# worldlife123/cbench_BaSIC

Hardware: AMD Instinct MI355X
Metric: encode+decode Mpix/s (higher is better)
Workload: dtype f32; 1 GPU; hyperprior codec N=128 M=192 (lossy_graph_scalable_exp_hp), synthetic 3x256x256 images (image i = manual_seed(i), rand), 256 images per GPU per step resident in HBM, compress+decompress incl. bitstream D2H/H2D, 6 concurrent stream workers per GPU (step k on worker k mod W: whole batches, W in flight); images_per_gpu=256, workers=6, rans_waves_per_workgroup=8, batches_in_flight=6, parallelism=image-sharded x1, RCCL all-reduce of metric sums

## Files before the change

### cbench_basic_amd/csrc/conv.hip

```cpp
#include "common.h"

#include <cstdlib>
#include <cstring>
#include <new>
#include <vector>

using namespace basic;

namespace {
thread_local bool g_dynamic_tiles = false;
}
namespace basic {
bool set_dynamic_tiles(bool on)
{
    const bool prev = g_dynamic_tiles;
    g_dynamic_tiles = on;
    return prev;
}
}

namespace {

typedef float f32x16 __attribute__((ext_vector_type(16)));
typedef float f32x4 __attribute__((ext_vector_type(4)));
// ... 1 lines not shown
constexpr int kFewTaps = 9;
constexpr int kVeryFewTaps = 6;
constexpr int stage_channels(int ntaps, int waves)
{
    return (ntaps > kFewTaps ? 2 : (ntaps > kVeryFewTaps ? 4 : 8)) * (waves == 8 ? 2 : 1);
}
constexpr int plan_waves(int mt, int ntaps) { return (mt == 4 && ntaps > kFewTaps) ? 8 : 4; }
constexpr int kMaxTaps = 25;
constexpr int kTilePos = 128;
constexpr int kPSlots = 12;
constexpr int kPSlotsNarrow = 24;
constexpr int patch_slots(int mt) { return mt <= 2 ? kPSlotsNarrow : kPSlots; }
constexpr int kPSlotsFused = 6;
constexpr int kFusedCK = 4;
constexpr int kMaxCoutPerLaunch = 192;
constexpr int kSplitBelowBlocks = 384;
constexpr int kPackTail = 32 * 32 * 8 + 2048;

struct TapLaunch {
    const float *in;
    float *out;
    const float *wpack;
    const float *wrow;
    const float *bias;
    int64_t split_wstride;
    const float *gammaT;
    const float *beta;
    int batch, cin, cin_pad, cout, coutp;
    int out_ctotal, co_base;
    int in_h, in_w, out_h, out_w;
// ... 325 lines not shown
            }
    }
}

typedef __bf16 bf16x8 __attribute__((ext_vector_type(8)));
typedef unsigned u32x4 __attribute__((ext_vector_type(4)));

constexpr int kSplitWaves = 8;
constexpr int kSplitThreads = 64 * kSplitWaves;
constexpr int kSplitCK = 16;
constexpr int kSplitStageTaps = 5;
constexpr int kSplitBlockU4 = 4 * 3 * 64;
constexpr int kSplitStageU4 = kSplitStageTaps * kSplitBlockU4;
constexpr int kSplitWSlots = (kSplitStageU4 + kSplitThreads - 1) / kSplitThreads;
static_assert(kSplitWSlots % 2 == 0, "weight stage in two halves");
constexpr size_t kSplitLdsBytes = 2 * kSplitStageU4 * 16 + 2 * 128 * sizeof(float);

__device__ __forceinline__ void split_bf16x3(const float (&x)[8], u32x4 &p0, u32x4 &p1, u32x4 &p2)
{
#pragma unroll
    for (int i = 0; i < 4; ++i) {
        const unsigned a = __float_as_uint(x[2 * i]), b = __float_as_uint(x[2 * i + 1]);
        const unsigned a0 = a & 0xFFFF0000u, b0 = b & 0xFFFF0000u;
        p0[i] = (a >> 16) | b0;
        const unsigned ra = __float_as_uint(x[2 * i] - __uint_as_float(a0)), rb = __float_as_uint(x[2 * i + 1] - __uint_as_float(b0));
        const unsigned a1 = ra & 0xFFFF0000u, b1 = rb & 0xFFFF0000u;
        p1[i] = (ra >> 16) | b1;
        const unsigned sa = __float_as_uint(__uint_as_float(ra) - __uint_as_float(a1)), sb = __float_as_uint(__uint_as_float(rb) - __uint_as_float(b1));
        p2[i] = (sa >> 16) | (sb & 0xFFFF0000u);
    }
}

__device__ __forceinline__ f32x16 mfma_bf16(const u32x4 &a, const u32x4 &b, const f32x16 &c)
{
    return __builtin_amdgcn_mfma_f32_32x32x16_bf16(__builtin_bit_cast(bf16x8, a), __builtin_bit_cast(bf16x8, b), c, 0, 0, 0);
}

constexpr int kSplitPatchPos = 416;
constexpr int kSplitPieceBytes = kSplitPatchPos * 32;
constexpr size_t kSplitLdsPatchBytes = kSplitLdsBytes + 3 * kSplitPieceBytes;
static_assert(kSplitLdsPatchBytes <= 160 * 1024, "patch beside the weight stages");
static_assert(kSplitLdsBytes % 16 == 0, "16-byte aligned patch");
constexpr int kSplitPatchRounds = (2 * kSplitPatchPos + kSplitThreads - 1) / kSplitThreads;

template <int KH, int KW, int KWB, bool PATCH>
__global__ __launch_bounds__(kSplitThreads, 1) void conv_split_bf16_kernel(const TapLaunch g, const u32x4 *wsplit)
{
    constexpr int MT = 4;
    constexpr int kTapsA = KH * KW, kTapsAll = KH * (KW + KWB);
    constexpr int kGroups = kTapsAll / kSplitStageTaps;
    static_assert(kTapsAll % kSplitStageTaps == 0, "taps per channel block must be whole stages");
    static_assert(KWB > 0 && KWB <= KW, "fused phases: second grid inside the first");
    extern __shared__ u32x4 lds_u4[];
    float *chan_const = reinterpret_cast<float *>(lds_u4 + 2 * kSplitStageU4);

    const int tid = threadIdx.x;
    const int lane = tid & 63;
    const int khalf = lane >> 5;
    const int wave = __builtin_amdgcn_readfirstlane(tid >> 6);

    int bid = xcd_tile(blockIdx.x, gridDim.x);
    const int tx_i = bid % g.tiles_x; bid /= g.tiles_x;
    const int ty_i = bid % g.tiles_y; bid /= g.tiles_y;
    const int TB = 1 << g.tb_log, TH = 1 << g.th_log, TW = 1 << g.tw_log;
    const int b0 = bid * TB, my0 = ty_i * TH, mx0 = tx_i * TW;
    struct Pos { int tb, my, mx; };
    auto pos_of = [&](int t) {
        const int qq = (t >> 6) * 32 + (t & 31);
        return Pos{qq >> (g.tw_log + g.th_log), my0 + ((qq >> g.tw_log) & (TH - 1)), mx0 + (qq & (TW - 1))};
    };
    const Pos lp = pos_of(tid);
    const int tb = lp.tb, b = b0 + lp.tb;

    if (tid < 128) {
        chan_const[tid] = g.bias ? g.bias[tid] : 0.f;
        chan_const[128 + tid] = g.beta ? g.beta[tid] : 1.f;
    }

    const int64_t plane = static_cast<int64_t>(g.in_h) * g.in_w;
    const int nimg = (g.batch - b0 < TB) ? g.batch - b0 : TB;
    const __amdgpu_buffer_rsrc_t rsrc = __builtin_amdgcn_make_buffer_rsrc(
        const_cast<float *>(g.in + static_cast<int64_t>(b0) * g.cin * plane), 0, static_cast<int>(nimg * g.cin * plane * 4), 0x00020000);
    const int gy_l = lp.my * g.s_in + g.dymin, gx_l = lp.mx * g.s_in + g.dxmin;
    const int lane_off = static_cast<int>((((static_cast<int64_t>(tb) * g.cin + 8 * khalf) * g.in_h + gy_l) * g.in_w + gx_l) * 4);
    constexpr int kSpanX = KW;
    static_assert(KH * kSpanX <= 32, "one validity bit per tap offset");
    unsigned vmask = 0;
    if (b < g.batch) {
#pragma unroll
        for (int dy = 0; dy < KH; ++dy)
#pragma unroll
            for (int dx = 0; dx < kSpanX; ++dx) {
                const int yy = gy_l + dy, xx = gx_l + dx;
                if (yy >= 0 && yy < g.in_h && xx >= 0 && xx < g.in_w) vmask |= 1u << (dy * kSpanX + dx);
            }
    }
    const int plane_bytes = static_cast<int>(plane * 4);
    auto tap_row = [](int t) { return t < kTapsA ? t / KW : (t - kTapsA) / KWB; };
    auto tap_col = [](int t) { return t < kTapsA ? t % KW : (t - kTapsA) % KWB + (KW - KWB); };
    auto load_b = [&](int cb, int T, float (&d)[8]) __attribute__((always_inline)) {
        const int dy = tap_row(T), dx = tap_col(T);
        const int voff = ((vmask >> (dy * kSpanX + dx)) & 1u) ? lane_off + (dy * g.in_w + dx) * 4 : 0x7FFFFFF0;
        const int soff = cb * kSplitCK * plane_bytes;
#pragma unroll
        for (int j = 0; j < 8; ++j)
            d[j] = __builtin_bit_cast(float, __builtin_amdgcn_raw_buffer_load_b32(rsrc, voff, soff + j * plane_bytes, 0));
    };

    const int ncb = g.cin / kSplitCK;
    constexpr int kHalf = kSplitWSlots / 2;
    u32x4 wst[kHalf];
    auto fetch_w = [&](int s, int h) __attribute__((always_inline)) {
        const u32x4 *src = wsplit + static_cast<int64_t>(s) * kSplitStageU4 + tid;
#pragma unroll
        for (int sl = h * kHalf; sl < (h + 1) * kHalf; ++sl)
            if (sl * kSplitThreads + tid < kSplitStageU4) wst[sl - h * kHalf] = src[sl * kSplitThreads];
    };
    auto store_w = [&](int buf, int h) __attribute__((always_inline)) {
        u32x4 *dst = lds_u4 + buf * kSplitStageU4 + tid;
#pragma unroll
        for (int sl = h * kHalf; sl < (h + 1) * kHalf; ++sl)
            if (sl * kSplitThreads + tid < kSplitStageU4) dst[sl * kSplitThreads] = wst[sl - h * kHalf];
    };

    char *const patch = reinterpret_cast<char *>(lds_u4) + kSplitLdsBytes;
    const int PW = TW + KW - 1, PH = TH + KH - 1, npos = TB * PH * PW;
    int pvoff[kSplitPatchRounds], brow[KH];
    if constexpr (PATCH) {
#pragma unroll
        for (int r = 0; r < kSplitPatchRounds; ++r) {
            const int i = r * kSplitThreads + tid, p = i >> 1, h = i & 1;
            const int prow = p / PW, x = p - prow * PW, img = prow / PH, row = prow - img * PH;
            const int gy = my0 + g.dymin + row, gx = mx0 + g.dxmin + x;
            const bool inside = i < 2 * npos && img < nimg && gy >= 0 && gy < g.in_h && gx >= 0 && gx < g.in_w;
            pvoff[r] = inside ? static_cast<int>((((static_cast<int64_t>(img) * g.cin + 8 * h) * g.in_h + gy) * g.in_w + gx) * 4)
                              : 0x7FFFFFF0;
        }
#pragma unroll
        for (int dy = 0; dy < KH; ++dy) brow[dy] = ((tb * PH + (lp.my - my0) + dy) * PW + (lp.mx - mx0)) * 32 + 16 * khalf;
    }
    float pf[kSplitPatchRounds][8];
    auto fetch_patch = [&](int cb) __attribute__((always_inline)) {
        const int soff = cb * kSplitCK * plane_bytes;
#pragma unroll
        for (int r = 0; r < kSplitPatchRounds; ++r)
#pragma unroll
            for (int j = 0; j < 8; ++j)
                pf[r][j] = __builtin_bit_cast(float, __builtin_amdgcn_raw_buffer_load_b32(rsrc, pvoff[r], soff + j * plane_bytes, 0));
    };
    auto store_patch = [&]() __attribute__((always_inline)) {
#pragma unroll
        for (int r = 0; r < kSplitPatchRounds; ++r)
            if (r * kSplitThreads + tid < 2 * npos) {
                u32x4 q[3];
                split_bf16x3(pf[r], q[0], q[1], q[2]);
#pragma unroll
                for (int pc = 0; pc < 3; ++pc)
                    *reinterpret_cast<u32x4 *>(patch + (r * kSplitThreads + tid) * 16 + pc * kSplitPieceBytes) = q[pc];
            }
    };
    auto read_b = [&](int T, u32x4 (&d)[3]) __attribute__((always_inline)) {
        const char *src = patch + brow[tap_row(T)] + 32 * tap_col(T);
#pragma unroll
        for (int pc = 0; pc < 3; ++pc) d[pc] = *reinterpret_cast<const u32x4 *>(src + pc * kSplitPieceBytes);
    };

    f32x16 acc[MT], acc2[MT];
#pragma unroll
    for (int m = 0; m < MT; ++m)
#pragma unroll
        for (int r = 0; r < 16; ++r) {
            acc[m][r] = 0.f;
            acc2[m][r] = 0.f;
        }

    float xb[8];
    u32x4 bq[2][3];
    if constexpr (PATCH) fetch_patch(0);
    else load_b(0, 0, xb);
    fetch_w(0, 0);
    store_w(0, 0);
    fetch_w(0, 1);
    store_w(0, 1);
    if constexpr (PATCH) store_patch();
    for (int cb = 0; cb < ncb; ++cb) {
#pragma unroll
        for (int gi = 0; gi < kGroups; ++gi) {
            const int s = cb * kGroups + gi;
            __syncthreads();
            const bool more = s + 1 < ncb * kGroups;
            if (more) fetch_w(s + 1, 0);
            __builtin_amdgcn_sched_barrier(0);
            const u32x4 *wl = lds_u4 + (s & 1) * kSplitStageU4 + lane;
#pragma unroll
            for (int tl = 0; tl < kSplitStageTaps; ++tl) {
                const int T = gi * kSplitStageTaps + tl;
                float xn[8];
                u32x4 bd[3];
                if constexpr (PATCH) {
                    if (T == 0) read_b(0, bq[0]);
                } else {
                    if (T + 1 < kTapsAll) load_b(cb, T + 1, xn);
                    else load_b(cb + 1 < ncb ? cb + 1 : cb, 0, xn);
                    __builtin_amdgcn_sched_barrier(0);
                    split_bf16x3(xb, bd[0], bd[1], bd[2]);
                }
                const u32x4 (&bp)[3] = PATCH ? bq[T & 1] : bd;
                f32x16 (&dst)[MT] = T < kTapsA ? acc : acc2;
                u32x4 ap[2][3];
#pragma unroll
                for (int pc = 0; pc < 3; ++pc) ap[0][pc] = wl[(tl * MT * 3 + pc) * 64];
#pragma unroll
                for (int m = 0; m < MT; ++m) {
                    const int cur = m & 1;
                    if (m + 1 < MT) {
#pragma unroll
                        for (int pc = 0; pc < 3; ++pc) ap[cur ^ 1][pc] = wl[((tl * MT + m + 1) * 3 + pc) * 64];
                    } else if constexpr (PATCH) {
                        if (T + 1 < kTapsAll) read_b(T + 1, bq[(T + 1) & 1]);
                    }
                    __builtin_amdgcn_sched_barrier(0);
                    dst[m] = mfma_bf16(ap[cur][2], bp[0], dst[m]);
                    dst[m] = mfma_bf16(ap[cur][1], bp[1], dst[m]);
                    dst[m] = mfma_bf16(ap[cur][0], bp[2], dst[m]);
                    dst[m] = mfma_bf16(ap[cur][1], bp[0], dst[m]);
                    dst[m] = mfma_bf16(ap[cur][0], bp[1], dst[m]);
                    dst[m] = mfma_bf16(ap[cur][0], bp[0], dst[m]);
                    __builtin_amdgcn_sched_barrier(0);
                }
                if constexpr (!PATCH) {
#pragma unroll
                    for (int j = 0; j < 8; ++j) xb[j] = xn[j];
                }
                if (tl == 1 && more) {
                    store_w((s + 1) & 1, 0);
                    fetch_w(s + 1, 1);
                    __builtin_amdgcn_sched_barrier(0);
                }
                if constexpr (PATCH) {
                    if (gi == 0 && tl == 1) {
                        fetch_patch(cb + 1 < ncb ? cb + 1 : cb);
                        __builtin_amdgcn_sched_barrier(0);
                    }
                }
                if (tl == 3 && more) store_w((s + 1) & 1, 1);
            }
        }
        if constexpr (PATCH) {
            if (cb + 1 < ncb) {
                __syncthreads();
                store_patch();
            }
        }
    }

    const int tid_e = wave * 64 + static_cast<int>(__lane_id());
    const int khalf_e = (tid_e >> 5) & 1, col_e = tid_e & 31;
    float *gl = reinterpret_cast<float *>(lds_u4);
    const bool gdn = g.act == BASIC_ACT_GDN || g.act == BASIC_ACT_IGDN;
    auto finish = [&](f32x16 (&acc)[MT]) __attribute__((always_inline)) {
        if (g.bias) {
#pragma unroll
            for (int m = 0; m < MT; ++m)
#pragma unroll
                for (int rq = 0; rq < 4; ++rq) {
                    const f32x4 b4 = *reinterpret_cast<const f32x4 *>(chan_const + 32 * m + 8 * rq + 4 * khalf_e);
#pragma unroll
                    for (int e = 0; e < 4; ++e) acc[m][4 * rq + e] += b4[e];
                }
        }
        if (gdn) {
            f32x16 nrm[MT];
#pragma unroll
            for (int m = 0; m < MT; ++m)
#pragma unroll
                for (int r = 0; r < 16; ++r) nrm[m][r] = 0.f;
#pragma unroll
            for (int st = 0; st < 64; ++st) {
                const int kk = 32 * (st >> 4) + 8 * ((st & 15) >> 2) + (st & 3);
                float gk[4];
                load_a<4>(gl + ((kk + 4 * khalf_e) * 32 + col_e) * 4, gk);
                const float x = acc[st >> 4][st & 15];
                const float bfrag = x * x;
#pragma unroll
                for (int m = 0; m < MT; ++m)
                    nrm[m] = __builtin_amdgcn_mfma_f32_32x32x2f32(gk[m], bfrag, nrm[m], 0, 0, 0);
            }
#pragma unroll
            for (int m = 0; m < MT; ++m)
#pragma unroll
                for (int rq = 0; rq < 4; ++rq) {
                    const f32x4 b4 = *reinterpret_cast<const f32x4 *>(chan_const + 128 + 32 * m + 8 * rq + 4 * khalf_e);
#pragma unroll
                    for (int e = 0; e < 4; ++e) {
                        const int r = 4 * rq + e;
                        const float nv = nrm[m][r] + b4[e];
                        acc[m][r] *= (g.act == BASIC_ACT_GDN) ? __builtin_amdgcn_rsqf(nv) : __builtin_amdgcn_sqrtf(nv);
                    }
                }
        }
    };
    if (gdn) {
        __syncthreads();
        const f32x4 *src = reinterpret_cast<const f32x4 *>(g.gammaT);
        f32x4 *dst = reinterpret_cast<f32x4 *>(gl);
#pragma unroll
        for (int sl = 0; sl < 128 * 32 * 4 / 4 / kSplitThreads; ++sl) dst[sl * kSplitThreads + tid_e] = src[sl * kSplitThreads + tid_e];
        __syncthreads();
    }
    finish(acc);
    finish(acc2);

    const Pos ep = pos_of(tid_e);
    const int my = ep.my, mx = ep.mx, be = b0 + ep.tb;
    if (my < g.mh && mx < g.mw && be < g.batch) {
        const int oy = my * g.s_out + g.oy0, ox = mx * g.s_out + g.ox0;
        const int64_t oplane = static_cast<int64_t>(g.out_h) * g.out_w;
        float *o = g.out + (static_cast<int64_t>(be) * g.out_ctotal + g.co_base) * oplane + static_cast<int64_t>(oy) * g.out_w + ox;
#pragma unroll
        for (int m = 0; m < MT; ++m)
#pragma unroll
            for (int r = 0; r < 16; ++r) {
                const int co = 32 * m + 8 * (r >> 2) + 4 * khalf_e + (r & 3);
                if (co < g.cout) {
                    f32x2 v2;
                    v2[0] = apply_act(acc[m][r], g.act);
                    v2[1] = apply_act(acc2[m][r], g.act);
                    *reinterpret_cast<f32x2 *>(o + co * oplane) = v2;
                }
            }
    }
}

template <int KH, bool PATCH>
hipError_t launch_split(const TapLaunch &g, const u32x4 *ws, int blocks, hipStream_t st)
{
    const hipError_t e = ensure_max_lds(reinterpret_cast<const void *>(conv_split_bf16_kernel<KH, 3, 2, PATCH>));
    if (e != hipSuccess) return e;
    hipLaunchKernelGGL((conv_split_bf16_kernel<KH, 3, 2, PATCH>), dim3(blocks), dim3(kSplitThreads),
                       PATCH ? kSplitLdsPatchBytes : kSplitLdsBytes, st, g, ws);
    return hipGetLastError();
}

constexpr int kFirstSlots = 10;

template <bool ROWS>
__global__ __launch_bounds__(512, 1) void conv5x5_cin4_gdn_persistent_kernel(const TapLaunch g, int ntiles, int *sched)
{
    extern __shared__ float lds[];
    constexpr int MT = 4, kCK = ROWS ? 3 : 4, KW = 5, kSteps = ROWS ? 5 * 8 : 25 * 2;
    constexpr int kWFloats = ROWS ? 80 * 32 * 4 : 25 * 4 * 32 * 4;
    constexpr int kGFloats = 128 * 32 * 4;
    float *wl = lds;
    float *gl = lds + kWFloats;
    const int tid = threadIdx.x;
// ... 940 lines not shown
        if (kh == 3 && kw == 3) return launch_one<MT, kFew, 3, 3, WF>(g, blocks, nsplit, lds_bytes, st);
        return launch_one<MT, kFew, 0, 0, WF>(g, blocks, nsplit, lds_bytes, st);
    }
    if (kh == 3 && kw == 2) return launch_one<MT, kVeryFew, 3, 2, WV>(g, blocks, nsplit, lds_bytes, st);
    if (kh == 2 && kw == 3) return launch_one<MT, kVeryFew, 2, 3, WV>(g, blocks, nsplit, lds_bytes, st);
    if (kh == 2 && kw == 2) return launch_one<MT, kVeryFew, 2, 2, WV>(g, blocks, nsplit, lds_bytes, st);
    return launch_one<MT, kVeryFew, 0, 0, WV>(g, blocks, nsplit, lds_bytes, st);
}

int ilog2(int v) { int l = 0; while ((1 << (l + 1)) <= v) ++l; return l; }
int pow2_ceil(int v) { int p = 1; while (p < v) p <<= 1; return p; }

}

namespace {
struct LaunchChoice { bool use_split, fuse_ok, bf16x3, split_patch; };
LaunchChoice choose_launches(const basic_conv_plan *p, int batch, int oh, int ow, const void *d_out)
{
    const int64_t pos_blocks = (static_cast<int64_t>(batch) * ((oh + p->s_out - 1) / p->s_out) * ((ow + p->s_out - 1) / p->s_out) + kTilePos - 1) / kTilePos;
    const char *dbg_env = getenv("BASIC_CONV_DEBUG");
    const int dbg = dbg_env ? atoi(dbg_env) : 0;
    LaunchChoice c;
    c.use_split = !p->split.empty() && !(dbg & 8) && (pos_blocks < kSplitBelowBlocks || (dbg & 4));
    c.fuse_ok = ow % 2 == 0 && (reinterpret_cast<uintptr_t>(d_out) & 7) == 0 && !(dbg & 512);
    const char *f32_env = getenv("BASIC_CONV_F32");
    c.bf16x3 = !(f32_env && atoi(f32_env) != 0);
    c.split_patch = !(dbg & 1024);
    return c;
}
}

extern "C" int basic_conv_plan_launches(const basic_conv_plan *p, int batch, int in_h, int in_w)
{
    int oh = 0, ow = 0;
    if (!p || batch < 1 || basic_conv_plan_out_hw(p, in_h, in_w, &oh, &ow)) return -1;
    if (p->d_wsm) return 1;
    const LaunchChoice c = choose_launches(p, batch, oh, ow, nullptr);
    int n = 0;
    for (const Chunk &ch : (c.use_split ? p->split : p->chunks))
        for (const Phase &ph : ((c.fuse_ok && !ch.fused.empty()) ? ch.fused : ch.phases)) {
            const int mh = (oh - ph.oy0 + p->s_out - 1) / p->s_out, mw = (ow - ph.ox0 + p->s_out - 1) / p->s_out;
            if (mh > 0 && mw > 0) ++n;
// ... 16 lines not shown
        g.tiles_x = (in_w + kSmTileW - 1) / kSmTileW;
        const int blocks = batch * g.tiles_y * g.tiles_x;
        const bool dma_ok = in_w % 4 == 0 && (reinterpret_cast<uintptr_t>(d_in) & 15) == 0;
        if (dma_ok && in_h >= 64) {
            g.tiles_y = (in_h + kSm2TileH - 1) / kSm2TileH;
            hipLaunchKernelGGL(deconv5s2_cout3_dma2_kernel, dim3(batch * g.tiles_y * g.tiles_x), dim3(256), 0, as_stream(hip_stream), g);
        } else if (dma_ok)
            hipLaunchKernelGGL(deconv5s2_cout3_dma_kernel, dim3(blocks), dim3(256), 0, as_stream(hip_stream), g);
        else
            hipLaunchKernelGGL(deconv5s2_cout3_kernel, dim3(blocks), dim3(256), 0, as_stream(hip_stream), g);
        BASIC_HIP_TRY(hipGetLastError());
        return BASIC_OK;
    }
    const LaunchChoice choice = choose_launches(p, batch, oh, ow, d_out);
    const bool use_split = choice.use_split, fuse_ok = choice.fuse_ok;
    for (const Chunk &ch : (use_split ? p->split : p->chunks))
    for (const Phase &ph : ((fuse_ok && !ch.fused.empty()) ? ch.fused : ch.phases)) {
        TapLaunch g{};
        g.in = d_in; g.out = d_out; g.wpack = ph.d_wpack; g.wrow = ph.d_wrow; g.split_wstride = ph.split_wstride; g.bias = ch.d_bias; g.gammaT = p->d_gammaT; g.beta = p->d_beta;
        g.batch = batch; g.cin = p->cin; g.cin_pad = ph.ntaps ? ph.cin_pad : 0; g.cout = ch.cout; g.coutp = ch.coutp; g.out_ctotal = p->cout; g.co_base = ch.co0;
        g.in_h = in_h; g.in_w = in_w; g.out_h = oh; g.out_w = ow;
        g.s_in = p->s_in; g.s_out = p->s_out; g.oy0 = ph.oy0; g.ox0 = ph.ox0;
        g.mh = (oh - ph.oy0 + p->s_out - 1) / p->s_out;
        g.mw = (ow - ph.ox0 + p->s_out - 1) / p->s_out;
        if (g.mh <= 0 || g.mw <= 0) continue;
        g.ntaps = ph.ntaps; g.dymin = ph.dymin; g.dxmin = ph.dxmin;
        std::memcpy(g.dy, ph.dy, sizeof(g.dy));
        std::memcpy(g.dx, ph.dx, sizeof(g.dx));
        g.act = p->act;
        const int kCK = ph.ck;
        if (choice.bf16x3 && ph.d_wsplit) {
            int tw = pow2_ceil(g.mw); if (tw > 16) tw = 16;
            int th = pow2_ceil(g.mh); if (th > kSplitWaves * 32 / tw) th = kSplitWaves * 32 / tw;
            const int tb = kSplitWaves * 32 / (tw * th);
            if (static_cast<int64_t>(tb) * p->cin * in_h * in_w * 4 < (1ll << 31)) {
                g.tw_log = ilog2(tw); g.th_log = ilog2(th); g.tb_log = ilog2(tb);
                g.tiles_y = (g.mh + th - 1) / th;
                g.tiles_x = (g.mw + tw - 1) / tw;
                const int blocks = ((batch + tb - 1) / tb) * g.tiles_y * g.tiles_x;
                hipStream_t st = as_stream(hip_stream);
                const u32x4 *ws = static_cast<const u32x4 *>(ph.d_wsplit);
                BASIC_REQUIRE(ph.kw == 3 && ph.kwb == 2 && (ph.kh == 3 || ph.kh == 2), "conv_forward: split-bf16 plan / kernel instantiation mismatch");
                const bool patch = choice.split_patch && g.s_in == 1 && tb * (th + ph.kh - 1) * (tw + ph.kw - 1) <= kSplitPatchPos;
                const hipError_t e = ph.kh == 3 ? (patch ? launch_split<3, true>(g, ws, blocks, st) : launch_split<3, false>(g, ws, blocks, st))
                                                : (patch ? launch_split<2, true>(g, ws, blocks, st) : launch_split<2, false>(g, ws, blocks, st));
                BASIC_HIP_TRY(e);
                continue;
            }
        }
        int tw = pow2_ceil(g.mw); if (tw > 16) tw = 16;
        const int threads = 64 * ph.waves, tile_pos = 32 * ph.waves;
        int th = pow2_ceil(g.mh); if (th > tile_pos / tw) th = tile_pos / tw;
        int tb = tile_pos / (tw * th);
        const bool first_layer_path = ch.mt == 4 && ch.nsplit == 1 && ph.waves == 8 && ph.kh == 5 && ph.kw == 5 &&
                                      ph.cin_pad == kCK && kCK == 4 && ch.cout == 128 && p->d_gammaT;
        g.ph = (th - 1) * g.s_in + ph.span_y;
        g.pw = (tw - 1) * g.s_in + ph.span_x;
        g.patch4 = (ph.waves == 8 && !first_layer_path && in_w % 4 == 0 && (reinterpret_cast<uintptr_t>(d_in) & 15) == 0) ? 1 : 0;
        g.pwp = g.patch4 ? (g.pw + 3 + 3) / 4 * 4 : (g.pw | 1);
        const int punit = g.patch4 ? 4 : 1;
// ... 18 lines not shown
        hipStream_t st = as_stream(hip_stream);
        if (first_layer_path) {
            const bool rows = ph.d_wrow != nullptr;
            const int patch_pad1 = (tb * (rows ? 3 : kCK) * g.ph * g.pwp + 511) / 512 * 512;
            const size_t lds1 = sizeof(float) * ((rows ? 10240 : 12800) + 16384 + 2 * static_cast<size_t>(patch_pad1) + 256 + 4);
            if (lds1 <= 160 * 1024 && patch_pad1 <= kFirstSlots * 512) {
                BASIC_HIP_TRY(ensure_max_lds(reinterpret_cast<const void *>(conv5x5_cin4_gdn_persistent_kernel<false>)));
                BASIC_HIP_TRY(ensure_max_lds(reinterpret_cast<const void *>(conv5x5_cin4_gdn_persistent_kernel<true>)));
                int dev = 0, cus = 256;
                (void)hipGetDevice(&dev);
                (void)hipDeviceGetAttribute(&cus, hipDeviceAttributeMultiprocessorCount, dev);
                const int grid = blocks < cus ? blocks : cus;
                int *sched = nullptr;
                if (g_dynamic_tiles) {
                    auto *pm = const_cast<basic_conv_plan *>(p);
                    if (!pm->d_sched) BASIC_HIP_TRY(hipMalloc(&pm->d_sched, sizeof(int)));
                    BASIC_HIP_TRY(hipMemsetAsync(pm->d_sched, 0, sizeof(int), st));
                    sched = pm->d_sched;
                }
                if (rows) hipLaunchKernelGGL(conv5x5_cin4_gdn_persistent_kernel<true>, dim3(grid), dim3(512), lds1, st, g, blocks, sched);
                else hipLaunchKernelGGL(conv5x5_cin4_gdn_persistent_kernel<false>, dim3(grid), dim3(512), lds1, st, g, blocks, sched);
                BASIC_HIP_TRY(hipGetLastError());
                continue;
            }
        }
        if (ph.kwb) {
            switch (ch.mt) {
                case 1: rc = launch_fused<1>(g, ph.kh, ph.kw, ph.kwb, ph.ck, ph.waves, blocks, ch.nsplit, lds_bytes, st); break;
                case 2: rc = launch_fused<2>(g, ph.kh, ph.kw, ph.kwb, ph.ck, ph.waves, blocks, ch.nsplit, lds_bytes, st); break;
                case 3: rc = launch_fused<3>(g, ph.kh, ph.kw, ph.kwb, ph.ck, ph.waves, blocks, ch.nsplit, lds_bytes, st); break;
                case 4: rc = launch_fused<4>(g, ph.kh, ph.kw, ph.kwb, ph.ck, ph.waves, blocks, ch.nsplit, lds_bytes, st); break;
// ... 19 lines not shown
```

Before: 827.6 Mpix/s.

## Make split-bf16 conv kernel persistent with atomic dynamic tile scheduling

Turns the split-bf16x3 conv kernel into a persistent kernel launched with at most one block per CU. Each block pulls further tiles through an atomic counter and prefetches the next tile's weights and patch across tile boundaries, so per-block launch and prologue costs are paid once per block rather than once per tile. Weight fetches move to buffer loads, and the LDS layout is reworked to hold a next-tile slot. The price is a memset and atomic counters per plan, shared mutable scheduler state that could race between concurrent streams using the same plan, and a more intricate pipeline.

```diff
diff --git a/cbench_basic_amd/csrc/conv.hip b/cbench_basic_amd/csrc/conv.hip
--- a/cbench_basic_amd/csrc/conv.hip
+++ b/cbench_basic_amd/csrc/conv.hip
@@ -39,6 +39,7 @@
 constexpr int kPSlotsFused = 6;
 constexpr int kFusedCK = 4;
 constexpr int kMaxCoutPerLaunch = 192;
+constexpr int kSchedCounters = 16;
 constexpr int kSplitBelowBlocks = 384;
 constexpr int kPackTail = 32 * 32 * 8 + 2048;
 
@@ -394,7 +395,13 @@
 constexpr int kSplitStageU4 = kSplitStageTaps * kSplitBlockU4;
 constexpr int kSplitWSlots = (kSplitStageU4 + kSplitThreads - 1) / kSplitThreads;
 static_assert(kSplitWSlots % 2 == 0, "weight stage in two halves");
-constexpr size_t kSplitLdsBytes = 2 * kSplitStageU4 * 16 + 2 * 128 * sizeof(float);
+constexpr int kSplitStageBytes = kSplitStageU4 * 16;
+constexpr int kSplitGammaOff = kSplitStageBytes;
+constexpr int kSplitGammaBytes = 128 * 32 * 4 * static_cast<int>(sizeof(float));
+constexpr int kSplitConstBytes = 2 * 128 * static_cast<int>(sizeof(float));
+constexpr int kSplitConstOffDirect = kSplitGammaOff + kSplitGammaBytes;
+constexpr int kSplitSlotOffDirect = kSplitConstOffDirect + kSplitConstBytes;
+constexpr size_t kSplitLdsBytes = kSplitSlotOffDirect + 16;
 
 __device__ __forceinline__ void split_bf16x3(const float (&x)[8], u32x4 &p0, u32x4 &p1, u32x4 &p2)
 {
@@ -418,13 +425,19 @@
 
 constexpr int kSplitPatchPos = 416;
 constexpr int kSplitPieceBytes = kSplitPatchPos * 32;
-constexpr size_t kSplitLdsPatchBytes = kSplitLdsBytes + 3 * kSplitPieceBytes;
+constexpr int kSplitPatchOff = 2 * kSplitStageBytes;
+constexpr int kSplitConstOffPatch = kSplitPatchOff + 3 * kSplitPieceBytes;
+constexpr int kSplitSlotOffPatch = kSplitConstOffPatch - 4;
+constexpr size_t kSplitLdsPatchBytes = kSplitConstOffPatch + kSplitConstBytes;
 static_assert(kSplitLdsPatchBytes <= 160 * 1024, "patch beside the weight stages");
-static_assert(kSplitLdsBytes % 16 == 0, "16-byte aligned patch");
+static_assert(kSplitPatchOff % 16 == 0, "16-byte aligned patch");
+static_assert(kSplitGammaOff + kSplitGammaBytes <= kSplitConstOffPatch, "gamma^T below bias and beta");
 constexpr int kSplitPatchRounds = (2 * kSplitPatchPos + kSplitThreads - 1) / kSplitThreads;
 
+typedef const __attribute__((address_space(4))) TapLaunch *SplitArgs;
+
 template <int KH, int KW, int KWB, bool PATCH>
-__global__ __launch_bounds__(kSplitThreads, 1) void conv_split_bf16_kernel(const TapLaunch g, const u32x4 *wsplit)
+__global__ __launch_bounds__(kSplitThreads, 1) void conv_split_bf16_kernel(const TapLaunch g, const u32x4 *wsplit, int ntiles, int *sched)
 {
     constexpr int MT = 4;
     constexpr int kTapsA = KH * KW, kTapsAll = KH * (KW + KWB);
@@ -432,55 +445,88 @@
     static_assert(kTapsAll % kSplitStageTaps == 0, "taps per channel block must be whole stages");
     static_assert(KWB > 0 && KWB <= KW, "fused phases: second grid inside the first");
     extern __shared__ u32x4 lds_u4[];
-    float *chan_const = reinterpret_cast<float *>(lds_u4 + 2 * kSplitStageU4);
+    char *const lds = reinterpret_cast<char *>(lds_u4);
+    float *chan_const = reinterpret_cast<float *>(lds + (PATCH ? kSplitConstOffPatch : kSplitConstOffDirect));
+    int *const next_slot = reinterpret_cast<int *>(lds + (PATCH ? kSplitSlotOffPatch : kSplitSlotOffDirect));
 
     const int tid = threadIdx.x;
-    const int lane = tid & 63;
-    const int khalf = lane >> 5;
     const int wave = __builtin_amdgcn_readfirstlane(tid >> 6);
-
-    int bid = xcd_tile(blockIdx.x, gridDim.x);
-    const int tx_i = bid % g.tiles_x; bid /= g.tiles_x;
-    const int ty_i = bid % g.tiles_y; bid /= g.tiles_y;
     const int TB = 1 << g.tb_log, TH = 1 << g.th_log, TW = 1 << g.tw_log;
-    const int b0 = bid * TB, my0 = ty_i * TH, mx0 = tx_i * TW;
-    struct Pos { int tb, my, mx; };
-    auto pos_of = [&](int t) {
-        const int qq = (t >> 6) * 32 + (t & 31);
-        return Pos{qq >> (g.tw_log + g.th_log), my0 + ((qq >> g.tw_log) & (TH - 1)), mx0 + (qq & (TW - 1))};
-    };
-    const Pos lp = pos_of(tid);
-    const int tb = lp.tb, b = b0 + lp.tb;
 
     if (tid < 128) {
         chan_const[tid] = g.bias ? g.bias[tid] : 0.f;
         chan_const[128 + tid] = g.beta ? g.beta[tid] : 1.f;
     }
-
+    if (tid == 0) *next_slot = static_cast<int>(gridDim.x) + atomicAdd(sched, 1);
+
+    int b0, my0, mx0;
+    struct Pos { int tb, my, mx; };
+    auto pos_of = [&](const auto &G, int t, int my0_, int mx0_) {
+        const int qq = (t >> 6) * 32 + (t & 31);
+        return Pos{qq >> (G.tw_log + G.th_log), my0_ + ((qq >> G.tw_log) & ((1 << G.th_log) - 1)), mx0_ + (qq & ((1 << G.tw_log) - 1))};
+    };
+    const int in_w = g.in_w;
     const int64_t plane = static_cast<int64_t>(g.in_h) * g.in_w;
-    const int nimg = (g.batch - b0 < TB) ? g.batch - b0 : TB;
-    const __amdgpu_buffer_rsrc_t rsrc = __builtin_amdgcn_make_buffer_rsrc(
-        const_cast<float *>(g.in + static_cast<int64_t>(b0) * g.cin * plane), 0, static_cast<int>(nimg * g.cin * plane * 4), 0x00020000);
-    const int gy_l = lp.my * g.s_in + g.dymin, gx_l = lp.mx * g.s_in + g.dxmin;
-    const int lane_off = static_cast<int>((((static_cast<int64_t>(tb) * g.cin + 8 * khalf) * g.in_h + gy_l) * g.in_w + gx_l) * 4);
+    const int plane_bytes = static_cast<int>(plane * 4);
+    __amdgpu_buffer_rsrc_t rsrc;
+    int lane_off;
     constexpr int kSpanX = KW;
     static_assert(KH * kSpanX <= 32, "one validity bit per tap offset");
-    unsigned vmask = 0;
-    if (b < g.batch) {
-#pragma unroll
-        for (int dy = 0; dy < KH; ++dy)
-#pragma unroll
-            for (int dx = 0; dx < kSpanX; ++dx) {
-                const int yy = gy_l + dy, xx = gx_l + dx;
-                if (yy >= 0 && yy < g.in_h && xx >= 0 && xx < g.in_w) vmask |= 1u << (dy * kSpanX + dx);
-            }
-    }
-    const int plane_bytes = static_cast<int>(plane * 4);
+    unsigned vmask;
+    char *const patch = lds + kSplitPatchOff;
+    const int PW = TW + KW - 1, PH = TH + KH - 1, npos = TB * PH * PW;
+    int pvoff[kSplitPatchRounds], brow[KH];
+    auto enter_tile = [&](const auto &G, int tile, int t) __attribute__((always_inline)) {
+        const int TB = 1 << G.tb_log, TH = 1 << G.th_log, TW = 1 << G.tw_log;
+        const int PW = TW + KW - 1, PH = TH + KH - 1, npos = TB * PH * PW;
+        const int64_t plane = static_cast<int64_t>(G.in_h) * G.in_w;
+        const int tx_i = tile % G.tiles_x; tile /= G.tiles_x;
+        const int ty_i = tile % G.tiles_y; tile /= G.tiles_y;
+        b0 = tile * TB; my0 = ty_i * TH; mx0 = tx_i * TW;
+        const Pos lp = pos_of(G, t, my0, mx0);
+        const int kh = (t >> 5) & 1;
+        const int nimg = (G.batch - b0 < TB) ? G.batch - b0 : TB;
+        rsrc = __builtin_amdgcn_make_buffer_rsrc(
+            const_cast<float *>(G.in + static_cast<int64_t>(b0) * G.cin * plane), 0, static_cast<int>(nimg * G.cin * plane * 4), 0x00020000);
+        const int gy_l = lp.my * G.s_in + G.dymin, gx_l = lp.mx * G.s_in + G.dxmin;
+        lane_off = static_cast<int>((((static_cast<int64_t>(lp.tb) * G.cin + 8 * kh) * G.in_h + gy_l) * G.in_w + gx_l) * 4);
+        vmask = 0;
+        if (b0 + lp.tb < G.batch) {
+#pragma unroll
+            for (int dy = 0; dy < KH; ++dy)
+#pragma unroll
+                for (int dx = 0; dx < kSpanX; ++dx) {
+                    const int yy = gy_l + dy, xx = gx_l + dx;
+                    if (yy >= 0 && yy < G.in_h && xx >= 0 && xx < G.in_w) vmask |= 1u << (dy * kSpanX + dx);
+                }
+        }
+        if constexpr (PATCH) {
+#pragma unroll
+            for (int r = 0; r < kSplitPatchRounds; ++r) {
+                const int i = r * kSplitThreads + t, p = i >> 1, h = i & 1;
+                const int prow = p / PW, x = p - prow * PW, img = prow / PH, row = prow - img * PH;
+                const int gy = my0 + G.dymin + row, gx = mx0 + G.dxmin + x;
+                const bool inside = i < 2 * npos && img < nimg && gy >= 0 && gy < G.in_h && gx >= 0 && gx < G.in_w;
+                pvoff[r] = inside ? static_cast<int>((((static_cast<int64_t>(img) * G.cin + 8 * h) * G.in_h + gy) * G.in_w + gx) * 4)
+                                  : 0x7FFFFFF0;
+            }
+        }
+    };
+    auto enter_tile_rows = [&](const auto &G, int t) __attribute__((always_inline)) {
+        if constexpr (PATCH) {
+            const int TH = 1 << G.th_log, TW = 1 << G.tw_log;
+            const int PW = TW + KW - 1, PH = TH + KH - 1;
+            const Pos lp = pos_of(G, t, 0, 0);
+#pragma unroll
+            for (int dy = 0; dy < KH; ++dy) brow[dy] = ((lp.tb * PH + lp.my + dy) * PW + lp.mx) * 32 + 16 * ((t >> 5) & 1);
+        }
+    };
+
     auto tap_row = [](int t) { return t < kTapsA ? t / KW : (t - kTapsA) / KWB; };
     auto tap_col = [](int t) { return t < kTapsA ? t % KW : (t - kTapsA) % KWB + (KW - KWB); };
     auto load_b = [&](int cb, int T, float (&d)[8]) __attribute__((always_inline)) {
         const int dy = tap_row(T), dx = tap_col(T);
-        const int voff = ((vmask >> (dy * kSpanX + dx)) & 1u) ? lane_off + (dy * g.in_w + dx) * 4 : 0x7FFFFFF0;
+        const int voff = ((vmask >> (dy * kSpanX + dx)) & 1u) ? lane_off + (dy * in_w + dx) * 4 : 0x7FFFFFF0;
         const int soff = cb * kSplitCK * plane_bytes;
 #pragma unroll
         for (int j = 0; j < 8; ++j)
@@ -488,13 +534,14 @@
     };
 
     const int ncb = g.cin / kSplitCK;
+    const int nst = ncb * kGroups;
     constexpr int kHalf = kSplitWSlots / 2;
+    const __amdgpu_buffer_rsrc_t wrsrc = __builtin_amdgcn_make_buffer_rsrc(const_cast<u32x4 *>(wsplit), 0, nst * kSplitStageBytes, 0x00020000);
     u32x4 wst[kHalf];
     auto fetch_w = [&](int s, int h) __attribute__((always_inline)) {
-        const u32x4 *src = wsplit + static_cast<int64_t>(s) * kSplitStageU4 + tid;
 #pragma unroll
         for (int sl = h * kHalf; sl < (h + 1) * kHalf; ++sl)
-            if (sl * kSplitThreads + tid < kSplitStageU4) wst[sl - h * kHalf] = src[sl * kSplitThreads];
+            wst[sl - h * kHalf] = __builtin_amdgcn_raw_buffer_load_b128(wrsrc, tid * 16, s * kSplitStageBytes + sl * kSplitThreads * 16, 0);
     };
     auto store_w = [&](int buf, int h) __attribute__((always_inline)) {
         u32x4 *dst = lds_u4 + buf * kSplitStageU4 + tid;
@@ -503,22 +550,6 @@
             if (sl * kSplitThreads + tid < kSplitStageU4) dst[sl * kSplitThreads] = wst[sl - h * kHalf];
     };
 
-    char *const patch = reinterpret_cast<char *>(lds_u4) + kSplitLdsBytes;
-    const int PW = TW + KW - 1, PH = TH + KH - 1, npos = TB * PH * PW;
-    int pvoff[kSplitPatchRounds], brow[KH];
-    if constexpr (PATCH) {
-#pragma unroll
-        for (int r = 0; r < kSplitPatchRounds; ++r) {
-            const int i = r * kSplitThreads + tid, p = i >> 1, h = i & 1;
-            const int prow = p / PW, x = p - prow * PW, img = prow / PH, row = prow - img * PH;
-            const int gy = my0 + g.dymin + row, gx = mx0 + g.dxmin + x;
-            const bool inside = i < 2 * npos && img < nimg && gy >= 0 && gy < g.in_h && gx >= 0 && gx < g.in_w;
-            pvoff[r] = inside ? static_cast<int>((((static_cast<int64_t>(img) * g.cin + 8 * h) * g.in_h + gy) * g.in_w + gx) * 4)
-                              : 0x7FFFFFF0;
-        }
-#pragma unroll
-        for (int dy = 0; dy < KH; ++dy) brow[dy] = ((tb * PH + (lp.my - my0) + dy) * PW + (lp.mx - mx0)) * 32 + 16 * khalf;
-    }
     float pf[kSplitPatchRounds][8];
     auto fetch_patch = [&](int cb) __attribute__((always_inline)) {
         const int soff = cb * kSplitCK * plane_bytes;
@@ -545,17 +576,11 @@
         for (int pc = 0; pc < 3; ++pc) d[pc] = *reinterpret_cast<const u32x4 *>(src + pc * kSplitPieceBytes);
     };
 
-    f32x16 acc[MT], acc2[MT];
-#pragma unroll
-    for (int m = 0; m < MT; ++m)
-#pragma unroll
-        for (int r = 0; r < 16; ++r) {
-            acc[m][r] = 0.f;
-            acc2[m][r] = 0.f;
-        }
-
     float xb[8];
     u32x4 bq[2][3];
+
+    enter_tile(g, xcd_tile(blockIdx.x, gridDim.x), tid);
+    enter_tile_rows(g, tid);
     if constexpr (PATCH) fetch_patch(0);
     else load_b(0, 0, xb);
     fetch_w(0, 0);
@@ -563,162 +588,219 @@
     fetch_w(0, 1);
     store_w(0, 1);
     if constexpr (PATCH) store_patch();
-    for (int cb = 0; cb < ncb; ++cb) {
-#pragma unroll
-        for (int gi = 0; gi < kGroups; ++gi) {
-            const int s = cb * kGroups + gi;
-            __syncthreads();
-            const bool more = s + 1 < ncb * kGroups;
-            if (more) fetch_w(s + 1, 0);
-            __builtin_amdgcn_sched_barrier(0);
-            const u32x4 *wl = lds_u4 + (s & 1) * kSplitStageU4 + lane;
-#pragma unroll
-            for (int tl = 0; tl < kSplitStageTaps; ++tl) {
-                const int T = gi * kSplitStageTaps + tl;
-                float xn[8];
-                u32x4 bd[3];
-                if constexpr (PATCH) {
-                    if (T == 0) read_b(0, bq[0]);
+
+    while (true) {
+        f32x16 acc[MT], acc2[MT];
+#pragma unroll
+        for (int m = 0; m < MT; ++m)
+#pragma unroll
+            for (int r = 0; r < 16; ++r) {
+                acc[m][r] = 0.f;
+                acc2[m][r] = 0.f;
+            }
+        int tile_next = 0;
+#pragma unroll 1
+        for (int cb = 0; cb < ncb; ++cb) {
+#pragma unroll
+            for (int gi = 0; gi < kGroups; ++gi) {
+                const int s = cb * kGroups + gi;
+                if (gi == 0 && cb == 0) {
+                    asm volatile("s_waitcnt lgkmcnt(0)" ::: "memory");
+                    __builtin_amdgcn_s_barrier();
+                    tile_next = __builtin_amdgcn_readfirstlane(*next_slot);
                 } else {
-                    if (T + 1 < kTapsAll) load_b(cb, T + 1, xn);
-                    else load_b(cb + 1 < ncb ? cb + 1 : cb, 0, xn);
-                    __builtin_amdgcn_sched_barrier(0);
-                    split_bf16x3(xb, bd[0], bd[1], bd[2]);
-                }
-                const u32x4 (&bp)[3] = PATCH ? bq[T & 1] : bd;
-                f32x16 (&dst)[MT] = T < kTapsA ? acc : acc2;
+                    __syncthreads();
+                }
+                const bool more = s + 1 < nst;
+                const bool fill = more || (tile_next < ntiles && (nst & 1) == 0);
+                const int sn = more ? s + 1 : 0;
+                if (fill) fetch_w(sn, 0);
+                __builtin_amdgcn_sched_barrier(0);
+                const u32x4 *wl = lds_u4 + (s & 1) * kSplitStageU4 + (tid & 63);
                 u32x4 ap[2][3];
 #pragma unroll
-                for (int pc = 0; pc < 3; ++pc) ap[0][pc] = wl[(tl * MT * 3 + pc) * 64];
-#pragma unroll
-                for (int m = 0; m < MT; ++m) {
-                    const int cur = m & 1;
-                    if (m + 1 < MT) {
-#pragma unroll
-                        for (int pc = 0; pc < 3; ++pc) ap[cur ^ 1][pc] = wl[((tl * MT + m + 1) * 3 + pc) * 64];
-                    } else if constexpr (PATCH) {
-                        if (T + 1 < kTapsAll) read_b(T + 1, bq[(T + 1) & 1]);
+                for (int tl = 0; tl < kSplitStageTaps; ++tl) {
+                    const int T = gi * kSplitStageTaps + tl;
+                    float xn[8];
+                    u32x4 bd[3];
+                    if constexpr (PATCH) {
+                        if (T == 0) read_b(0, bq[0]);
+                    } else {
+                        if (T + 1 < kTapsAll) load_b(cb, T + 1, xn);
+                        else load_b(cb + 1 < ncb ? cb + 1 : cb, 0, xn);
+                        __builtin_amdgcn_sched_barrier(0);
+                        split_bf16x3(xb, bd[0], bd[1], bd[2]);
                     }
-                    __builtin_amdgcn_sched_barrier(0);
-                    dst[m] = mfma_bf16(ap[cur][2], bp[0], dst[m]);
-                    dst[m] = mfma_bf16(ap[cur][1], bp[1], dst[m]);
-                    dst[m] = mfma_bf16(ap[cur][0], bp[2], dst[m]);
-                    dst[m] = mfma_bf16(ap[cur][1], bp[0], dst[m]);
-                    dst[m] = mfma_bf16(ap[cur][0], bp[1], dst[m]);
-                    dst[m] = mfma_bf16(ap[cur][0], bp[0], dst[m]);
-                    __builtin_amdgcn_sched_barrier(0);
-                }
-                if constexpr (!PATCH) {
-#pragma unroll
-                    for (int j = 0; j < 8; ++j) xb[j] = xn[j];
-                }
-                if (tl == 1 && more) {
-                    store_w((s + 1) & 1, 0);
-                    fetch_w(s + 1, 1);
-                    __builtin_amdgcn_sched_barrier(0);
-                }
-                if constexpr (PATCH) {
-                    if (gi == 0 && tl == 1) {
-                        fetch_patch(cb + 1 < ncb ? cb + 1 : cb);
+                    const u32x4 (&bp)[3] = PATCH ? bq[T & 1] : bd;
+                    f32x16 (&dst)[MT] = T < kTapsA ? acc : acc2;
+                    if (tl == 0) {
+#pragma unroll
+                        for (int pc = 0; pc < 3; ++pc) ap[0][pc] = wl[pc * 64];
+                    }
+#pragma unroll
+                    for (int m = 0; m < MT; ++m) {
+                        const int cur = m & 1;
+                        if (m + 1 < MT) {
+#pragma unroll
+                            for (int pc = 0; pc < 3; ++pc) ap[cur ^ 1][pc] = wl[((tl * MT + m + 1) * 3 + pc) * 64];
+                        } else {
+                            if (tl + 1 < kSplitStageTaps) {
+#pragma unroll
+                                for (int pc = 0; pc < 3; ++pc) ap[0][pc] = wl[((tl + 1) * MT * 3 + pc) * 64];
+                            }
+                            if constexpr (PATCH) {
+                                if (T + 1 < kTapsAll) read_b(T + 1, bq[(T + 1) & 1]);
+                            }
+                        }
+                        __builtin_amdgcn_sched_barrier(0);
+                        dst[m] = mfma_bf16(ap[cur][2], bp[0], dst[m]);
+                        dst[m] = mfma_bf16(ap[cur][1], bp[1], dst[m]);
+                        dst[m] = mfma_bf16(ap[cur][0], bp[2], dst[m]);
+                        dst[m] = mfma_bf16(ap[cur][1], bp[0], dst[m]);
+                        dst[m] = mfma_bf16(ap[cur][0], bp[1], dst[m]);
+                        dst[m] = mfma_bf16(ap[cur][0], bp[0], dst[m]);
                         __builtin_amdgcn_sched_barrier(0);
                     }
-                }
-                if (tl == 3 && more) store_w((s + 1) & 1, 1);
-            }
-        }
-        if constexpr (PATCH) {
-            if (cb + 1 < ncb) {
-                __syncthreads();
-                store_patch();
-            }
-        }
-    }
-
-    const int tid_e = wave * 64 + static_cast<int>(__lane_id());
-    const int khalf_e = (tid_e >> 5) & 1, col_e = tid_e & 31;
-    float *gl = reinterpret_cast<float *>(lds_u4);
-    const bool gdn = g.act == BASIC_ACT_GDN || g.act == BASIC_ACT_IGDN;
-    auto finish = [&](f32x16 (&acc)[MT]) __attribute__((always_inline)) {
-        if (g.bias) {
+                    if constexpr (!PATCH) {
+#pragma unroll
+                        for (int j = 0; j < 8; ++j) xb[j] = xn[j];
+                    }
+                    if (tl == 1 && fill) {
+                        store_w((s + 1) & 1, 0);
+                        fetch_w(sn, 1);
+                        __builtin_amdgcn_sched_barrier(0);
+                    }
+                    if constexpr (PATCH) {
+                        if (gi == 0 && tl == 1) {
+                            fetch_patch(cb + 1 < ncb ? cb + 1 : cb);
+                            __builtin_amdgcn_sched_barrier(0);
+                        }
+                    }
+                    if (tl == 3 && fill) store_w((s + 1) & 1, 1);
+                }
+            }
+            if constexpr (PATCH) {
+                if (cb + 1 < ncb) {
+                    __syncthreads();
+                    store_patch();
+                }
+            }
+        }
+
+        int tid_e = wave * 64 + static_cast<int>(__lane_id());
+        asm volatile("" : "+v"(tid_e));
+        SplitArgs ge = (SplitArgs)__builtin_amdgcn_kernarg_segment_ptr();
+        asm volatile("" : "+s"(ge));
+        const int khalf_e = (tid_e >> 5) & 1, col_e = tid_e & 31;
+        float *gl = reinterpret_cast<float *>(lds + kSplitGammaOff);
+        const bool gdn = ge->act == BASIC_ACT_GDN || ge->act == BASIC_ACT_IGDN;
+        const bool have_next = tile_next < ntiles;
+        const bool carried = have_next && (nst & 1) == 0;
+        auto finish = [&](f32x16 (&acc)[MT]) __attribute__((always_inline)) {
+            if (ge->bias) {
+#pragma unroll
+                for (int m = 0; m < MT; ++m)
+#pragma unroll
+                    for (int rq = 0; rq < 4; ++rq) {
+                        const f32x4 b4 = *reinterpret_cast<const f32x4 *>(chan_const + 32 * m + 8 * rq + 4 * khalf_e);
+#pragma unroll
+                        for (int e = 0; e < 4; ++e) acc[m][4 * rq + e] += b4[e];
+                    }
+            }
+            if (gdn) {
+                f32x16 nrm[MT];
+#pragma unroll
+                for (int m = 0; m < MT; ++m)
+#pragma unroll
+                    for (int r = 0; r < 16; ++r) nrm[m][r] = 0.f;
+#pragma unroll
+                for (int st = 0; st < 64; ++st) {
+                    const int kk = 32 * (st >> 4) + 8 * ((st & 15) >> 2) + (st & 3);
+                    float gk[4];
+                    load_a<4>(gl + ((kk + 4 * khalf_e) * 32 + col_e) * 4, gk);
+                    const float x = acc[st >> 4][st & 15];
+                    const float bfrag = x * x;
+#pragma unroll
+                    for (int m = 0; m < MT; ++m)
+                        nrm[m] = __builtin_amdgcn_mfma_f32_32x32x2f32(gk[m], bfrag, nrm[m], 0, 0, 0);
+                }
+#pragma unroll
+                for (int m = 0; m < MT; ++m)
+#pragma unroll
+                    for (int rq = 0; rq < 4; ++rq) {
+                        const f32x4 b4 = *reinterpret_cast<const f32x4 *>(chan_const + 128 + 32 * m + 8 * rq + 4 * khalf_e);
+#pragma unroll
+                        for (int e = 0; e < 4; ++e) {
+                            const int r = 4 * rq + e;
+                            const float nv = nrm[m][r] + b4[e];
+                            acc[m][r] *= (ge->act == BASIC_ACT_GDN) ? __builtin_amdgcn_rsqf(nv) : __builtin_amdgcn_sqrtf(nv);
+                        }
+                    }
+            }
+        };
+        int tile_after = 0;
+        if (have_next && tid_e == 0) tile_after = static_cast<int>(gridDim.x) + atomicAdd(sched, 1);
+        if (gdn) {
+            __syncthreads();
+            const __amdgpu_buffer_rsrc_t grsrc = __builtin_amdgcn_make_buffer_rsrc(const_cast<float *>(ge->gammaT), 0, kSplitGammaBytes, 0x00020000);
+            u32x4 *dst = reinterpret_cast<u32x4 *>(gl);
+#pragma unroll
+            for (int sl = 0; sl < kSplitGammaBytes / 16 / kSplitThreads; ++sl)
+                dst[sl * kSplitThreads + tid_e] = __builtin_amdgcn_raw_buffer_load_b128(grsrc, tid_e * 16, sl * kSplitThreads * 16, 0);
+        }
+        if (have_next && tid_e == 0) *next_slot = tile_after;
+        if (gdn) __syncthreads();
+        const int eb0 = b0, emy0 = my0, emx0 = mx0;
+        if (have_next) {
+            enter_tile(*ge, tile_next, tid_e);
+            if constexpr (PATCH) fetch_patch(0);
+            else load_b(0, 0, xb);
+        }
+        finish(acc);
+        finish(acc2);
+        asm volatile("s_waitcnt lgkmcnt(0)" ::: "memory");
+        __builtin_amdgcn_s_barrier();
+        if (have_next) {
+            if (!carried) {
+                fetch_w(0, 0);
+                store_w(0, 0);
+                fetch_w(0, 1);
+                store_w(0, 1);
+            }
+            if constexpr (PATCH) store_patch();
+            enter_tile_rows(*ge, tid_e);
+        }
+
+        const Pos ep = pos_of(*ge, tid_e, emy0, emx0);
+        const int my = ep.my, mx = ep.mx, be = eb0 + ep.tb;
+        if (my < ge->mh && mx < ge->mw && be < ge->batch) {
+            const int oy = my * ge->s_out + ge->oy0, ox = mx * ge->s_out + ge->ox0;
+            const int64_t oplane = static_cast<int64_t>(ge->out_h) * ge->out_w;
+            float *o = ge->out + (static_cast<int64_t>(be) * ge->out_ctotal + ge->co_base) * oplane + static_cast<int64_t>(oy) * ge->out_w + ox;
 #pragma unroll
             for (int m = 0; m < MT; ++m)
 #pragma unroll
-                for (int rq = 0; rq < 4; ++rq) {
-                    const f32x4 b4 = *reinterpret_cast<const f32x4 *>(chan_const + 32 * m + 8 * rq + 4 * khalf_e);
-#pragma unroll
-                    for (int e = 0; e < 4; ++e) acc[m][4 * rq + e] += b4[e];
-                }
-        }
-        if (gdn) {
-            f32x16 nrm[MT];
-#pragma unroll
-            for (int m = 0; m < MT; ++m)
-#pragma unroll
-                for (int r = 0; r < 16; ++r) nrm[m][r] = 0.f;
-#pragma unroll
-            for (int st = 0; st < 64; ++st) {
-                const int kk = 32 * (st >> 4) + 8 * ((st & 15) >> 2) + (st & 3);
-                float gk[4];
-                load_a<4>(gl + ((kk + 4 * khalf_e) * 32 + col_e) * 4, gk);
-                const float x = acc[st >> 4][st & 15];
-                const float bfrag = x * x;
-#pragma unroll
-                for (int m = 0; m < MT; ++m)
-                    nrm[m] = __builtin_amdgcn_mfma_f32_32x32x2f32(gk[m], bfrag, nrm[m], 0, 0, 0);
-            }
-#pragma unroll
-            for (int m = 0; m < MT; ++m)
-#pragma unroll
-                for (int rq = 0; rq < 4; ++rq) {
-                    const f32x4 b4 = *reinterpret_cast<const f32x4 *>(chan_const + 128 + 32 * m + 8 * rq + 4 * khalf_e);
-#pragma unroll
-                    for (int e = 0; e < 4; ++e) {
-                        const int r = 4 * rq + e;
-                        const float nv = nrm[m][r] + b4[e];
-                        acc[m][r] *= (g.act == BASIC_ACT_GDN) ? __builtin_amdgcn_rsqf(nv) : __builtin_amdgcn_sqrtf(nv);
+                for (int r = 0; r < 16; ++r) {
+                    const int co = 32 * m + 8 * (r >> 2) + 4 * khalf_e + (r & 3);
+                    if (co < ge->cout) {
+                        f32x2 v2;
+                        v2[0] = apply_act(acc[m][r], ge->act);
+                        v2[1] = apply_act(acc2[m][r], ge->act);
+                        *reinterpret_cast<f32x2 *>(o + co * oplane) = v2;
                     }
                 }
         }
-    };
-    if (gdn) {
-        __syncthreads();
-        const f32x4 *src = reinterpret_cast<const f32x4 *>(g.gammaT);
-        f32x4 *dst = reinterpret_cast<f32x4 *>(gl);
-#pragma unroll
-        for (int sl = 0; sl < 128 * 32 * 4 / 4 / kSplitThreads; ++sl) dst[sl * kSplitThreads + tid_e] = src[sl * kSplitThreads + tid_e];
-        __syncthreads();
-    }
-    finish(acc);
-    finish(acc2);
-
-    const Pos ep = pos_of(tid_e);
-    const int my = ep.my, mx = ep.mx, be = b0 + ep.tb;
-    if (my < g.mh && mx < g.mw && be < g.batch) {
-        const int oy = my * g.s_out + g.oy0, ox = mx * g.s_out + g.ox0;
-        const int64_t oplane = static_cast<int64_t>(g.out_h) * g.out_w;
-        float *o = g.out + (static_cast<int64_t>(be) * g.out_ctotal + g.co_base) * oplane + static_cast<int64_t>(oy) * g.out_w + ox;
-#pragma unroll
-        for (int m = 0; m < MT; ++m)
-#pragma unroll
-            for (int r = 0; r < 16; ++r) {
-                const int co = 32 * m + 8 * (r >> 2) + 4 * khalf_e + (r & 3);
-                if (co < g.cout) {
-                    f32x2 v2;
-                    v2[0] = apply_act(acc[m][r], g.act);
-                    v2[1] = apply_act(acc2[m][r], g.act);
-                    *reinterpret_cast<f32x2 *>(o + co * oplane) = v2;
-                }
-            }
+        if (!have_next) break;
     }
 }
 
 template <int KH, bool PATCH>
-hipError_t launch_split(const TapLaunch &g, const u32x4 *ws, int blocks, hipStream_t st)
+hipError_t launch_split(const TapLaunch &g, const u32x4 *ws, int tiles, int grid, int *sched, hipStream_t st)
 {
     const hipError_t e = ensure_max_lds(reinterpret_cast<const void *>(conv_split_bf16_kernel<KH, 3, 2, PATCH>));
     if (e != hipSuccess) return e;
-    hipLaunchKernelGGL((conv_split_bf16_kernel<KH, 3, 2, PATCH>), dim3(blocks), dim3(kSplitThreads),
-                       PATCH ? kSplitLdsPatchBytes : kSplitLdsBytes, st, g, ws);
+    hipLaunchKernelGGL((conv_split_bf16_kernel<KH, 3, 2, PATCH>), dim3(grid), dim3(kSplitThreads),
+                       PATCH ? kSplitLdsPatchBytes : kSplitLdsBytes, st, g, ws, tiles, sched);
     return hipGetLastError();
 }
 
@@ -1689,7 +1771,7 @@
 }
 
 namespace {
-struct LaunchChoice { bool use_split, fuse_ok, bf16x3, split_patch; };
+struct LaunchChoice { bool use_split, fuse_ok, bf16x3, split_patch; int split_grid; };
 LaunchChoice choose_launches(const basic_conv_plan *p, int batch, int oh, int ow, const void *d_out)
 {
     const int64_t pos_blocks = (static_cast<int64_t>(batch) * ((oh + p->s_out - 1) / p->s_out) * ((ow + p->s_out - 1) / p->s_out) + kTilePos - 1) / kTilePos;
@@ -1701,6 +1783,7 @@
     const char *f32_env = getenv("BASIC_CONV_F32");
     c.bf16x3 = !(f32_env && atoi(f32_env) != 0);
     c.split_patch = !(dbg & 1024);
+    c.split_grid = (dbg & 4096) ? -1 : (dbg & 2048) ? 2 : 0;
     return c;
 }
 }
@@ -1747,6 +1830,7 @@
     }
     const LaunchChoice choice = choose_launches(p, batch, oh, ow, d_out);
     const bool use_split = choice.use_split, fuse_ok = choice.fuse_ok;
+    int split_launches = 0;
     for (const Chunk &ch : (use_split ? p->split : p->chunks))
     for (const Phase &ph : ((fuse_ok && !ch.fused.empty()) ? ch.fused : ch.phases)) {
         TapLaunch g{};
@@ -1770,13 +1854,23 @@
                 g.tw_log = ilog2(tw); g.th_log = ilog2(th); g.tb_log = ilog2(tb);
                 g.tiles_y = (g.mh + th - 1) / th;
                 g.tiles_x = (g.mw + tw - 1) / tw;
-                const int blocks = ((batch + tb - 1) / tb) * g.tiles_y * g.tiles_x;
+                const int tiles = ((batch + tb - 1) / tb) * g.tiles_y * g.tiles_x;
                 hipStream_t st = as_stream(hip_stream);
                 const u32x4 *ws = static_cast<const u32x4 *>(ph.d_wsplit);
                 BASIC_REQUIRE(ph.kw == 3 && ph.kwb == 2 && (ph.kh == 3 || ph.kh == 2), "conv_forward: split-bf16 plan / kernel instantiation mismatch");
-                const bool patch = choice.split_patch && g.s_in == 1 && tb * (th + ph.kh - 1) * (tw + ph.kw - 1) <= kSplitPatchPos;
-                const hipError_t e = ph.kh == 3 ? (patch ? launch_split<3, true>(g, ws, blocks, st) : launch_split<3, false>(g, ws, blocks, st))
-                                                : (patch ? launch_split<2, true>(g, ws, blocks, st) : launch_split<2, false>(g, ws, blocks, st));
+                const bool patch = choice.split_patch && g.s_in == 1 && tb * (th + ph.kh - 1) * (tw + ph.kw - 1) < kSplitPatchPos;
+                int dev = 0, cus = 256;
+                (void)hipGetDevice(&dev);
+                (void)hipDeviceGetAttribute(&cus, hipDeviceAttributeMultiprocessorCount, dev);
+                const int cap = choice.split_grid < 0 ? tiles : choice.split_grid > 0 ? choice.split_grid : cus;
+                const int grid = tiles < cap ? tiles : cap;
+                BASIC_REQUIRE(split_launches < kSchedCounters, "conv_forward: more split-bf16 launches than tile counters");
+                auto *pm = const_cast<basic_conv_plan *>(p);
+                if (!pm->d_sched) BASIC_HIP_TRY(hipMalloc(&pm->d_sched, kSchedCounters * sizeof(int)));
+                if (split_launches == 0) BASIC_HIP_TRY(hipMemsetAsync(pm->d_sched, 0, kSchedCounters * sizeof(int), st));
+                int *sched = pm->d_sched + split_launches++;
+                const hipError_t e = ph.kh == 3 ? (patch ? launch_split<3, true>(g, ws, tiles, grid, sched, st) : launch_split<3, false>(g, ws, tiles, grid, sched, st))
+                                                : (patch ? launch_split<2, true>(g, ws, tiles, grid, sched, st) : launch_split<2, false>(g, ws, tiles, grid, sched, st));
                 BASIC_HIP_TRY(e);
                 continue;
             }
@@ -1825,7 +1919,7 @@
                 int *sched = nullptr;
                 if (g_dynamic_tiles) {
                     auto *pm = const_cast<basic_conv_plan *>(p);
-                    if (!pm->d_sched) BASIC_HIP_TRY(hipMalloc(&pm->d_sched, sizeof(int)));
+                    if (!pm->d_sched) BASIC_HIP_TRY(hipMalloc(&pm->d_sched, kSchedCounters * sizeof(int)));
                     BASIC_HIP_TRY(hipMemsetAsync(pm->d_sched, 0, sizeof(int), st));
                     sched = pm->d_sched;
                 }
```

Result: slower. 787.0 Mpix/s (-4.9%).
